# kevalmorabia97/CoVA-Web-Object-Detection

Hardware: AMD Instinct MI355X
Metric: webpages/sec fwd+bwd (90 bboxes, K=24) (higher is better)
Workload: dtype f32

## Files before the change

### cova-web-object-detection_amd/csrc/bn.hip

```cpp
#include "common.h"
#include "bn_tail.h"

namespace {

__device__ __forceinline__ int pow2_cols(int C)
{
    int cb = 1;
    while (cb < C && cb < 256) cb <<= 1;
    return cb;
}
inline int pow2_cols_host(int C)
{
    int cb = 1;
    while (cb < C && cb < 256) cb <<= 1;
    return cb;
}

template <int MODE>
__global__ __launch_bounds__(256) void colreduce_kernel(
    const float *__restrict__ x, int ldx, const float *__restrict__ act, int lda,
    const float *__restrict__ z, int ldz, const float *__restrict__ mean,
    const float *__restrict__ invstd, float *__restrict__ partial, long long R, int C,
    int rows_per_chunk)
{
// ... 180 lines not shown
        if (dbeta) dbeta[c] = (float)s1;
        if (dgamma) dgamma[c] = (float)s2;
        coef[c] = (float)(s1 / count);
        coef[C + c] = (float)(s2 / count);
    }
}

__global__ __launch_bounds__(1024) void bn_finalize_bwd_abc_kernel(
    const float *__restrict__ partial, int nparts, int C, double count,
    float *__restrict__ dgamma, float *__restrict__ dbeta, const float *__restrict__ mean,
    const float *__restrict__ invstd, const float *__restrict__ scale, float *__restrict__ abc)
{
    __shared__ double s_a[1024], s_b[1024];
    const int c = blockIdx.x * 64 + (threadIdx.x & 63), slice = threadIdx.x >> 6;
    double s1, s2;
    combine_partials(partial, nparts, C, c, slice, s_a, s_b, s1, s2);
    if (slice == 0 && c < C) bn_bwd_abc_channel(s1, s2, count, c, C, dgamma, dbeta, mean, invstd, scale, abc);
}

template <int V>
__global__ __launch_bounds__(256) void bn_act_fwd_kernel(
    const float *__restrict__ z, int ldz, const float *__restrict__ scale,
    const float *__restrict__ shift, const float *__restrict__ res, int ldres,
    float *__restrict__ out, int ldo, long long R, int C, int relu)
{
    const int CV = C / V;
    const long long total = R * CV;
    for (long long i = (long long)blockIdx.x * blockDim.x + threadIdx.x; i < total;
         i += (long long)gridDim.x * blockDim.x) {
        const long long r = i / CV;
        const int c = (int)(i - r * CV) * V;
        float v[V], sc[V], sh[V], rr[V];
        if (V == 4) {
            *reinterpret_cast<float4 *>(v) = *reinterpret_cast<const float4 *>(z + r * ldz + c);
            *reinterpret_cast<float4 *>(sc) = *reinterpret_cast<const float4 *>(scale + c);
            *reinterpret_cast<float4 *>(sh) = *reinterpret_cast<const float4 *>(shift + c);
            if (res) *reinterpret_cast<float4 *>(rr) = *reinterpret_cast<const float4 *>(res + r * ldres + c);
        } else {
            v[0] = z[r * ldz + c]; sc[0] = scale[c]; sh[0] = shift[c];
            if (res) rr[0] = res[r * ldres + c];
        }
#pragma unroll
        for (int j = 0; j < V; ++j) {
            float y = fmaf(sc[j], v[j], sh[j]);
            if (res) y += rr[j];
            if (relu) y = y > 0.f ? y : 0.f;
            v[j] = y;
        }
        if (V == 4) *reinterpret_cast<float4 *>(out + r * ldo + c) = *reinterpret_cast<float4 *>(v);
        else out[r * ldo + c] = v[0];
    }
}

template <int U>
__global__ __launch_bounds__(256) void bn_act_fwd_bits_kernel(
    const float *__restrict__ z, const float *__restrict__ scale, const float *__restrict__ shift,
    const float *__restrict__ res, float *__restrict__ out, uint32_t *__restrict__ bits, long long R)
{
    const long long total = R * 16;
    const long long stride = (long long)gridDim.x * blockDim.x;
    const int c = (int)(threadIdx.x & 15) * 4;
    const float4 sc = *reinterpret_cast<const float4 *>(scale + c), sh = *reinterpret_cast<const float4 *>(shift + c);
    for (long long i0 = (long long)blockIdx.x * blockDim.x + threadIdx.x; i0 < total; i0 += stride * U) {
      float4 vv[U], rr[U];
#pragma unroll
      for (int u = 0; u < U; ++u) {
        const long long i = i0 + u * stride;
        const long long ic = i < total ? i : i0;
        vv[u] = *reinterpret_cast<const float4 *>(z + ic * 4);
        if (res != nullptr) rr[u] = *reinterpret_cast<const float4 *>(res + ic * 4);
      }
#pragma unroll
      for (int u = 0; u < U; ++u) {
        const long long i = i0 + u * stride;
        if (i >= total) break;
        const float4 v = vv[u];
        float y[4] = {fmaf(sc.x, v.x, sh.x), fmaf(sc.y, v.y, sh.y), fmaf(sc.z, v.z, sh.z), fmaf(sc.w, v.w, sh.w)};
        if (res != nullptr) {
            const float4 r4 = rr[u];
            y[0] += r4.x; y[1] += r4.y; y[2] += r4.z; y[3] += r4.w;
        }
        uint32_t word = 0u;
#pragma unroll
        for (int j = 0; j < 4; ++j) {
            y[j] = y[j] > 0.f ? y[j] : 0.f;
            word |= (y[j] > 0.f ? 1u : 0u) << j;
        }
        *reinterpret_cast<float4 *>(out + i * 4) = make_float4(y[0], y[1], y[2], y[3]);
        word <<= 4 * (threadIdx.x & 7);
        word |= __shfl_xor(word, 1, 64);
        word |= __shfl_xor(word, 2, 64);
        word |= __shfl_xor(word, 4, 64);
        if ((threadIdx.x & 7) == 0) bits[i >> 3] = word;
      }
    }
}

__global__ __launch_bounds__(256) void bn_act2_fwd_kernel(
    const float *__restrict__ z, const float *__restrict__ scale, const float *__restrict__ shift,
    const float *__restrict__ z2, const float *__restrict__ scale2, const float *__restrict__ shift2,
    float *__restrict__ out, long long R, int C, int relu)
{
    const int CV = C / 4;
    const long long total = R * CV;
    for (long long i = (long long)blockIdx.x * blockDim.x + threadIdx.x; i < total;
         i += (long long)gridDim.x * blockDim.x) {
        const int c = (int)(i % CV) * 4;
        const float4 a = *reinterpret_cast<const float4 *>(z + i * 4);
        const float4 b = *reinterpret_cast<const float4 *>(z2 + i * 4);
        const float4 sa = *reinterpret_cast<const float4 *>(scale + c), ha = *reinterpret_cast<const float4 *>(shift + c);
        const float4 sb = *reinterpret_cast<const float4 *>(scale2 + c), hb = *reinterpret_cast<const float4 *>(shift2 + c);
        float4 y;
        y.x = fmaf(sa.x, a.x, ha.x) + fmaf(sb.x, b.x, hb.x);
        y.y = fmaf(sa.y, a.y, ha.y) + fmaf(sb.y, b.y, hb.y);
        y.z = fmaf(sa.z, a.z, ha.z) + fmaf(sb.z, b.z, hb.z);
        y.w = fmaf(sa.w, a.w, ha.w) + fmaf(sb.w, b.w, hb.w);
        if (relu) {
            y.x = y.x > 0.f ? y.x : 0.f; y.y = y.y > 0.f ? y.y : 0.f;
            y.z = y.z > 0.f ? y.z : 0.f; y.w = y.w > 0.f ? y.w : 0.f;
        }
        *reinterpret_cast<float4 *>(out + i * 4) = y;
    }
}

template <int V>
__global__ __launch_bounds__(256) void bn_bwd_apply_kernel(
    const float *__restrict__ dout, int ldd, const float *__restrict__ act, int lda,
    const float *__restrict__ z, int ldz, const float *__restrict__ mean,
    const float *__restrict__ invstd, const float *__restrict__ scale,
    const float *__restrict__ coef, float *__restrict__ dz, int lddz, float *__restrict__ dres,
    int lddres, long long R, int C)
{
    const int CV = C / V;
    const long long total = R * CV;
    for (long long i = (long long)blockIdx.x * blockDim.x + threadIdx.x; i < total;
         i += (long long)gridDim.x * blockDim.x) {
        const long long r = i / CV;
        const int c = (int)(i - r * CV) * V;
        float g[V], a[V], zz[V], o[V];
        if (V == 4) {
            *reinterpret_cast<float4 *>(g) = *reinterpret_cast<const float4 *>(dout + r * ldd + c);
            *reinterpret_cast<float4 *>(zz) = *reinterpret_cast<const float4 *>(z + r * ldz + c);
            if (act) *reinterpret_cast<float4 *>(a) = *reinterpret_cast<const float4 *>(act + r * lda + c);
        } else {
            g[0] = dout[r * ldd + c]; zz[0] = z[r * ldz + c];
            if (act) a[0] = act[r * lda + c];
        }
#pragma unroll
        for (int j = 0; j < V; ++j) {
            float dy = g[j];
            if (act && !(a[j] > 0.f)) dy = 0.f;
            g[j] = dy;
            const float xh = (zz[j] - mean[c + j]) * invstd[c + j];
            o[j] = scale[c + j] * (dy - coef[c + j] - xh * coef[C + c + j]);
        }
        if (V == 4) {
            *reinterpret_cast<float4 *>(dz + r * lddz + c) = *reinterpret_cast<float4 *>(o);
            if (dres) *reinterpret_cast<float4 *>(dres + r * lddres + c) = *reinterpret_cast<float4 *>(g);
        } else {
            dz[r * lddz + c] = o[0];
            if (dres) dres[r * lddres + c] = g[0];
        }
    }
}

template <bool XCD>
__global__ __launch_bounds__(256) void bn_relu_maxpool_fwd_kernel(
    const float *__restrict__ y, const float *__restrict__ scale, const float *__restrict__ shift,
    float *__restrict__ out, uint8_t *__restrict__ idx, float *__restrict__ ymax, int B, int H1, int W1,
    int H2, int W2)
{
    constexpr int POOL_STRIP = 1;
    const int nstrips = (H2 + POOL_STRIP - 1) / POOL_STRIP;
    const long long total = (long long)B * nstrips * W2 * 16;
    long long wb = blockIdx.x;
    if (XCD) {
        const long long per = gridDim.x / 8;
        if (wb < per * 8) wb = (wb % 8) * per + wb / 8;
    }
    for (long long i = wb * blockDim.x + threadIdx.x; i < total; i += (long long)gridDim.x * blockDim.x) {
        const int c4 = (int)(i & 15);
        long long p = i >> 4;
        const int ox = (int)(p % W2);
        p /= W2;
        const int strip = (int)(p % nstrips), b = (int)(p / nstrips);
        const float4 sc = *reinterpret_cast<const float4 *>(scale + c4 * 4);
        const float4 sh = *reinterpret_cast<const float4 *>(shift + c4 * 4);
        const float scv[4] = {sc.x, sc.y, sc.z, sc.w}, shv[4] = {sh.x, sh.y, sh.z, sh.w};
        const float *yb = y + (size_t)b * H1 * W1 * 64 + c4 * 4;
        const int ix0 = 2 * ox - 1;
        const bool okx[3] = {ix0 >= 0, true, ix0 + 2 < W1};
        auto load_row = [&](int iy, float4 (&r)[3]) {
#pragma unroll
            for (int kx = 0; kx < 3; ++kx) {
                const int ix = min(max(ix0 + kx, 0), W1 - 1), iyc = min(max(iy, 0), H1 - 1);
                r[kx] = *reinterpret_cast<const float4 *>(yb + ((size_t)iyc * W1 + ix) * 64);
            }
        };
        const int oy0 = strip * POOL_STRIP, oy1 = min(oy0 + POOL_STRIP, H2);
        float4 top[3], mid[3], bot[3];
        load_row(2 * oy0 - 1, top);
        for (int oy = oy0; oy < oy1; ++oy) {
            load_row(2 * oy, mid);
            load_row(2 * oy + 1, bot);
            const bool oky[3] = {2 * oy - 1 >= 0, true, 2 * oy + 1 < H1};
            float m[4] = {-INFINITY, -INFINITY, -INFINITY, -INFINITY};
            float my[4] = {0.f, 0.f, 0.f, 0.f};
            int mi[4] = {0, 0, 0, 0};
#pragma unroll
            for (int ky = 0; ky < 3; ++ky) {
                const float4 *row = ky == 0 ? top : ky == 1 ? mid : bot;
#pragma unroll
                for (int kx = 0; kx < 3; ++kx) {
                    if (!(oky[ky] && okx[kx])) continue;
                    const float vv[4] = {row[kx].x, row[kx].y, row[kx].z, row[kx].w};
#pragma unroll
                    for (int j = 0; j < 4; ++j) {
                        const float t = fmaf(vv[j], scv[j], shv[j]);
                        const float a = t > 0.f ? t : 0.f;
                        if (a > m[j]) { m[j] = a; mi[j] = ky * 3 + kx; my[j] = vv[j]; }
                    }
                }
            }
            const size_t o = (((size_t)b * H2 + oy) * W2 + ox) * 64 + c4 * 4;
            *reinterpret_cast<float4 *>(out + o) = make_float4(m[0], m[1], m[2], m[3]);
            *reinterpret_cast<uchar4 *>(idx + o) = make_uchar4(mi[0], mi[1], mi[2], mi[3]);
            if (ymax != nullptr) *reinterpret_cast<float4 *>(ymax + o) = make_float4(my[0], my[1], my[2], my[3]);
#pragma unroll
            for (int kx = 0; kx < 3; ++kx) top[kx] = bot[kx];
        }
    }
}

__global__ __launch_bounds__(256) void bn_relu_maxpool_bwd_reduce_win_kernel(
    const float *__restrict__ dp, const uint8_t *__restrict__ idx, const float *__restrict__ y,
    const float *__restrict__ scale, const float *__restrict__ shift,
    const float *__restrict__ mean, const float *__restrict__ invstd, float *__restrict__ partial,
    int B, int H1, int W1, int H2, int W2)
{
    __shared__ float s_s[16][64], s_q[16][64];
    const int c4 = threadIdx.x & 15, prow = threadIdx.x >> 4;
    const float4 sc = *reinterpret_cast<const float4 *>(scale + c4 * 4);
    const float4 sh = *reinterpret_cast<const float4 *>(shift + c4 * 4);
    const float4 mu = *reinterpret_cast<const float4 *>(mean + c4 * 4);
    const float4 is = *reinterpret_cast<const float4 *>(invstd + c4 * 4);
    const float scv[4] = {sc.x, sc.y, sc.z, sc.w}, shv[4] = {sh.x, sh.y, sh.z, sh.w};
    const float muv[4] = {mu.x, mu.y, mu.z, mu.w}, isv[4] = {is.x, is.y, is.z, is.w};
    float s[4] = {0, 0, 0, 0}, q[4] = {0, 0, 0, 0};
    const long long nwin = (long long)B * H2 * W2;
    for (long long p = (long long)blockIdx.x * 16 + prow; p < nwin; p += (long long)gridDim.x * 16) {
        const int ox = (int)(p % W2);
        const long long pr = p / W2;
        const int oy = (int)(pr % H2);
        const int b = (int)(pr / H2);
        const uchar4 id = *reinterpret_cast<const uchar4 *>(idx + (size_t)p * 64 + c4 * 4);
        const float4 g = *reinterpret_cast<const float4 *>(dp + (size_t)p * 64 + c4 * 4);
        const int pos[4] = {id.x, id.y, id.z, id.w};
        const float gv[4] = {g.x, g.y, g.z, g.w};
        const float *yb = y + (size_t)b * H1 * W1 * 64 + c4 * 4;
#pragma unroll
        for (int j = 0; j < 4; ++j) {
            const int ky = pos[j] / 3, kx = pos[j] - ky * 3;
            const int iy = 2 * oy - 1 + ky, ix = 2 * ox - 1 + kx;
            const float yv = yb[((size_t)iy * W1 + ix) * 64 + j];
            const float t = fmaf(yv, scv[j], shv[j]);
            const float dy = t > 0.f ? gv[j] : 0.f;
            s[j] += dy;
            q[j] += dy * ((yv - muv[j]) * isv[j]);
        }
    }
#pragma unroll
    for (int j = 0; j < 4; ++j) { s_s[prow][c4 * 4 + j] = s[j]; s_q[prow][c4 * 4 + j] = q[j]; }
    __syncthreads();
    if (threadIdx.x < 64) {
        float a = 0.f, bq = 0.f;
        for (int r = 0; r < 16; ++r) { a += s_s[r][threadIdx.x]; bq += s_q[r][threadIdx.x]; }
        partial[((size_t)blockIdx.x * 2 + 0) * 64 + threadIdx.x] = a;
        partial[((size_t)blockIdx.x * 2 + 1) * 64 + threadIdx.x] = bq;
// ... 119 lines not shown
                       (const float *)nullptr, 0, (const float *)nullptr, 0, (const float *)nullptr,
                       (const float *)nullptr, partial, R, C, rpc);
    COVA_LAUNCH_CHECK();
    return COVA_OK;
}

COVA_API int cova_bn_finalize_fwd(const float *partial, int nparts, int C, double count,
                                  const float *gamma, const float *beta, float *running_mean,
                                  float *running_var, long long *num_batches_tracked, float momentum,
                                  float eps, float *scale, float *shift, float *mean, float *invstd,
                                  void *stream)
{
    COVA_REQUIRE(partial && gamma && beta && scale && shift && mean && invstd && nparts > 0 && C > 0);
    hipLaunchKernelGGL(bn_finalize_fwd_kernel, dim3(cdiv(C, 64)), dim3(1024), 0, (hipStream_t)stream,
                       partial, nparts, C, count, gamma, beta, running_mean, running_var, momentum,
                       eps, scale, shift, mean, invstd, num_batches_tracked);
    COVA_LAUNCH_CHECK();
    return COVA_OK;
}

COVA_API int cova_bn_eval_params(const float *gamma, const float *beta, const float *running_mean,
                                 const float *running_var, float eps, int C, float *scale,
                                 float *shift, float *mean, float *invstd, void *stream)
{
    COVA_REQUIRE(gamma && beta && running_mean && running_var && scale && shift && C > 0);
    hipLaunchKernelGGL(bn_eval_params_kernel, dim3(cdiv(C, 256)), dim3(256), 0, (hipStream_t)stream,
                       gamma, beta, running_mean, running_var, eps, C, scale, shift, mean, invstd);
    COVA_LAUNCH_CHECK();
    return COVA_OK;
}

COVA_API int cova_bn_act_fwd(const float *z, int ldz, const float *scale, const float *shift,
                             const float *res, int ldres, float *out, int ldo, long long R, int C,
                             int relu, void *stream)
{
    COVA_REQUIRE(z && scale && shift && out && R > 0 && C > 0);
    const bool v4 = (C % 4 == 0) && vec4_ok(z, ldz) && vec4_ok(res, ldres) && vec4_ok(out, ldo) &&
                    vec4_ok(scale, 0) && vec4_ok(shift, 0);
    if (v4)
        hipLaunchKernelGGL(bn_act_fwd_kernel<4>, dim3(ew_grid(R * (C / 4))), dim3(256), 0,
                           (hipStream_t)stream, z, ldz, scale, shift, res, ldres, out, ldo, R, C, relu);
    else
        hipLaunchKernelGGL(bn_act_fwd_kernel<1>, dim3(ew_grid(R * C)), dim3(256), 0,
                           (hipStream_t)stream, z, ldz, scale, shift, res, ldres, out, ldo, R, C, relu);
    COVA_LAUNCH_CHECK();
    return COVA_OK;
}

COVA_API int cova_bn_act_fwd_bits(const float *z, const float *scale, const float *shift, const float *res, float *out,
                                  uint32_t *bits, long long R, void *stream)
{
    COVA_REQUIRE(z && scale && shift && out && bits && R > 0);
    COVA_REQUIRE(vec4_ok(z, 64) && vec4_ok(res, 64) && vec4_ok(out, 64) && vec4_ok(scale, 0) && vec4_ok(shift, 0));
    hipLaunchKernelGGL(bn_act_fwd_bits_kernel<1>, dim3(ew_grid(R * 16)), dim3(256), 0, (hipStream_t)stream, z, scale, shift,
                       res, out, bits, R);
    COVA_LAUNCH_CHECK();
    return COVA_OK;
}

COVA_API int cova_bn_act2_fwd(const float *z, const float *scale, const float *shift, const float *z2,
                              const float *scale2, const float *shift2, float *out, long long R, int C,
                              int relu, void *stream)
{
    COVA_REQUIRE(z && scale && shift && z2 && scale2 && shift2 && out && R > 0 && C > 0 && C % 4 == 0);
    COVA_REQUIRE(vec4_ok(z, C) && vec4_ok(z2, C) && vec4_ok(out, C) && vec4_ok(scale, 0) && vec4_ok(shift, 0) &&
                 vec4_ok(scale2, 0) && vec4_ok(shift2, 0));
    hipLaunchKernelGGL(bn_act2_fwd_kernel, dim3(ew_grid(R * (C / 4))), dim3(256), 0, (hipStream_t)stream, z,
                       scale, shift, z2, scale2, shift2, out, R, C, relu);
    COVA_LAUNCH_CHECK();
    return COVA_OK;
}

COVA_API int cova_bn_bwd_reduce(const float *dout, int ldd, const float *act, int lda,
                                const float *z, int ldz, const float *mean, const float *invstd,
                                long long R, int C, float *partial, void *stream)
{
    COVA_REQUIRE(dout && z && mean && invstd && partial && R > 0 && C > 0);
    const int rpc = cova_colreduce_rows_per_chunk(R, C);
    const dim3 grid((unsigned)cdivll(R, rpc), (unsigned)cdiv(C, pow2_cols_host(C)));
    if (C == 64 && ldd == 64 && ldz == 64 && (act == nullptr || lda == 64) && vec4_ok(dout, ldd) &&
        vec4_ok(z, ldz) && vec4_ok(act, lda)) {
        hipLaunchKernelGGL(colreduce64_kernel<1>, dim3(grid.x), dim3(256), 0, (hipStream_t)stream, dout,
                           act, z, mean, invstd, partial, R, rpc);
        COVA_LAUNCH_CHECK();
        return COVA_OK;
    }
    hipLaunchKernelGGL(colreduce_kernel<1>, grid, dim3(256), 0, (hipStream_t)stream, dout, ldd, act,
                       lda, z, ldz, mean, invstd, partial, R, C, rpc);
    COVA_LAUNCH_CHECK();
    return COVA_OK;
}

COVA_API int cova_bn_finalize_bwd(const float *partial, int nparts, int C, double count,
                                  float *dgamma, float *dbeta, float *coef, void *stream)
{
    COVA_REQUIRE(partial && coef && nparts > 0 && C > 0);
    hipLaunchKernelGGL(bn_finalize_bwd_kernel, dim3(cdiv(C, 64)), dim3(1024), 0, (hipStream_t)stream,
                       partial, nparts, C, count, dgamma, dbeta, coef);
    COVA_LAUNCH_CHECK();
    return COVA_OK;
}

COVA_API int cova_bn_finalize_bwd_abc(const float *partial, int nparts, int C, double count,
                                      float *dgamma, float *dbeta, const float *mean,
                                      const float *invstd, const float *scale, float *abc,
                                      void *stream)
{
    COVA_REQUIRE(partial && mean && invstd && scale && abc && nparts > 0 && C > 0);
    hipLaunchKernelGGL(bn_finalize_bwd_abc_kernel, dim3(cdiv(C, 64)), dim3(1024), 0,
                       (hipStream_t)stream, partial, nparts, C, count, dgamma, dbeta, mean, invstd,
                       scale, abc);
    COVA_LAUNCH_CHECK();
    return COVA_OK;
}

COVA_API int cova_bn_bwd_apply(const float *dout, int ldd, const float *act, int lda, const float *z,
                               int ldz, const float *mean, const float *invstd, const float *scale,
                               const float *coef, float *dz, int lddz, float *dres, int lddres,
                               long long R, int C, void *stream)
{
    COVA_REQUIRE(dout && z && mean && invstd && scale && coef && dz && R > 0 && C > 0);
    const bool v4 = (C % 4 == 0) && vec4_ok(dout, ldd) && vec4_ok(act, lda) && vec4_ok(z, ldz) &&
                    vec4_ok(dz, lddz) && vec4_ok(dres, lddres);
    if (v4)
        hipLaunchKernelGGL(bn_bwd_apply_kernel<4>, dim3(ew_grid(R * (C / 4))), dim3(256), 0,
                           (hipStream_t)stream, dout, ldd, act, lda, z, ldz, mean, invstd, scale,
                           coef, dz, lddz, dres, lddres, R, C);
    else
        hipLaunchKernelGGL(bn_bwd_apply_kernel<1>, dim3(ew_grid(R * C)), dim3(256), 0,
                           (hipStream_t)stream, dout, ldd, act, lda, z, ldz, mean, invstd, scale,
                           coef, dz, lddz, dres, lddres, R, C);
    COVA_LAUNCH_CHECK();
    return COVA_OK;
}

COVA_API int cova_bn_relu_maxpool_fwd(const float *y, const float *scale, const float *shift,
                                      float *out, uint8_t *idx, float *ymax, int B, int H1, int W1,
                                      void *stream)
{
    COVA_REQUIRE(y && scale && shift && out && idx && B > 0 && H1 > 0 && W1 > 0);
    const int H2 = (H1 + 2 - 3) / 2 + 1, W2 = (W1 + 2 - 3) / 2 + 1;
    long long g = cdivll((long long)B * H2 * W2 * 16, 256);
    if (g > 0x7fffffffll) g = 0x7fffffffll;
    hipLaunchKernelGGL(bn_relu_maxpool_fwd_kernel<true>, dim3((unsigned)g), dim3(256), 0, (hipStream_t)stream, y, scale, shift,
                       out, idx, ymax, B, H1, W1, H2, W2);
    COVA_LAUNCH_CHECK();
    return COVA_OK;
}

COVA_API int cova_bn_relu_maxpool_bwd_num_partials(int B, int H1, int W1)
{
    long long g = cdivll((long long)B * H1 * W1, 16 * 64);
    if (g > 4096) g = 4096;
    if (g < 1) g = 1;
    return (int)g;
}

COVA_API int cova_bn_relu_maxpool_bwd_reduce(const float *dp, const uint8_t *idx, const float *y,
                                             const float *scale, const float *shift,
                                             const float *mean, const float *invstd, float *partial,
                                             int B, int H1, int W1, void *stream)
{
    COVA_REQUIRE(dp && idx && y && scale && shift && mean && invstd && partial);
    const int H2 = (H1 + 2 - 3) / 2 + 1, W2 = (W1 + 2 - 3) / 2 + 1;
    const int grid = cova_bn_relu_maxpool_bwd_num_partials(B, H1, W1);
    hipLaunchKernelGGL(bn_relu_maxpool_bwd_reduce_win_kernel, dim3(grid), dim3(256), 0,
                       (hipStream_t)stream, dp, idx, y, scale, shift, mean, invstd, partial, B, H1, W1,
                       H2, W2);
    COVA_LAUNCH_CHECK();
    return COVA_OK;
}

COVA_API int cova_bn_relu_maxpool_bwd_apply(const float *dp, const uint8_t *idx, const float *y,
                                            const float *scale, const float *shift,
                                            const float *mean, const float *invstd,
                                            const float *coef, float *dz, int B, int H1, int W1,
                                            void *stream)
{
    COVA_REQUIRE(dp && idx && y && scale && shift && mean && invstd && coef && dz);
    const int H2 = (H1 + 2 - 3) / 2 + 1, W2 = (W1 + 2 - 3) / 2 + 1;
    const int grid = ew_grid((long long)B * H2 * W2 * 16);
    hipLaunchKernelGGL(bn_relu_maxpool_bwd_apply_quad_kernel, dim3(grid), dim3(256), 0,
                       (hipStream_t)stream, dp, idx, y, scale, shift, mean, invstd, coef, dz, B, H1, W1,
                       H2, W2);
    COVA_LAUNCH_CHECK();
    return COVA_OK;
}
```

### cova-web-object-detection_amd/engine.py

```python
import ctypes
import os

import torch

from . import _lib
from .weights import BACKBONE_CHANNELS as C64, CONTEXT_LAYERS, head_layout

GAT_MAX_K = 1024

call, query = _lib.call, _lib.query
BN_MOMENTUM, BN_EPS, LEAKY_SLOPE = 0.1, 1e-5, 0.2


DROPOUT_KEYS = ("decoder.0", "decoder.3")
ATTN_DROP_KEY = "attn_drop"
PAGE_ATTN_DROP_KEY = "page_attention.attn_drop"
PAGE_ENC_DROP_KEY = "page_encoder.drop"


def is_train(training, key):
    if isinstance(training, bool):
        return training
    if hasattr(training, "get"):
        return bool(training.get(key, True))
# ... 287 lines not shown
        self.c = c

    @property
    def ptr(self):
        return ctypes.addressof(self.c)


class Options:
    overlap_allreduce = os.environ.get("COVA_OVERLAP_ALLREDUCE", "1") != "0"
    bn_tail = os.environ.get("COVA_BN_TAIL", "1") != "0"


OPTIONS = Options()

CONV3_KEYS = ["convnet.4.0.conv1", "convnet.4.0.conv2", "convnet.4.1.conv1", "convnet.4.1.conv2"]
BN3_KEYS = ["convnet.4.0.bn1.", "convnet.4.0.bn2.", "convnet.4.1.bn1.", "convnet.4.1.bn2."]


class LazyFeature:
    __slots__ = ("z", "x", "scale", "shift", "shape")

    def __init__(self, z, x, scale, shift):
        self.z, self.x, self.scale, self.shift, self.shape = z, x, scale, shift, tuple(z.shape)


def is_bottleneck(params):
    return "convnet.4.0.conv3.weight" in params


@on_device_of(0)
def convstack_fwd(images, params, buffers, training, save=True, lazy_out=False):
    _check(images)
    B, _, H, W = images.shape
    H1, W1 = query("cova_conv_out_size", H, 7, 2, 3), query("cova_conv_out_size", W, 7, 2, 3)
    H2, W2 = query("cova_conv_out_size", H1, 3, 2, 1), query("cova_conv_out_size", W1, 3, 2, 1)
    bottleneck = is_bottleneck(params)
    layer2 = has_layer2(params)
    lazy_out = lazy_out and not layer2
    sv = {"images": images, "dims": (B, H, W, H1, W1, H2, W2), "kind": "bottleneck" if bottleneck else "basic"}
    if bottleneck:
        sv["_w3"] = conv3_weights([params["convnet.4.%d.conv2.weight" % b] for b in (0, 1, 2)], images)
    else:
        sv["_w3"] = conv3_weights([params[k + ".weight"] for k in CONV3_KEYS], images)
    y1 = _empty((B, H1, W1, C64), images)
    nt1 = query("cova_conv1_num_partials", B, H, W)
    stem_train = is_train(training, "convnet.1.")
    part = _empty((nt1, 2, C64), images) if stem_train else None
    if stem_train and tails_on():
        bn1, tail = bn_tail_fwd("convnet.1.", params, buffers, C64, images, B * H1 * W1)
        call("cova_conv1_fwd_tail", images, params["convnet.0.weight"], y1, part, B, H, W, tail.ptr)
    else:
        call("cova_conv1_fwd_tail", images, params["convnet.0.weight"], y1, part, B, H, W, None)
        bn1 = bn_params("convnet.1.", params, buffers, C64, images, training, part, nt1, B * H1 * W1, unit="pages")
    p1 = _empty((B, H2, W2, C64), images)
    idx = _empty((B, H2, W2, C64), images, torch.uint8)
    want_ymax = save and (stem_train or bottleneck)
    ymax = _empty((B, H2, W2, C64), images) if want_ymax else None
    call("cova_bn_relu_maxpool_fwd", y1, bn1.scale, bn1.shift, p1, idx, ymax, B, H1, W1)
    sv.update(y1=y1, bn1=bn1, idx=idx, ymax=ymax)
    if bottleneck:
        feat = _layer1_bottleneck_fwd(p1, params, buffers, training, save, lazy_out, sv)
    else:
        feat = _layer1_basic_fwd(p1, params, buffers, training, save, lazy_out, sv)
    if layer2:
        feat = _layer2_fwd(feat, params, buffers, training, save, sv)
    return feat, (sv if save else None)


def conv3_num_partials(B, H, W):
    return query("cova_conv3x3_wino4_num_partials", B, H, W)


def conv3x3_pro(u, inp, in2, abc, relu, addend, act, msc, msh, z, mean, invstd, out, part, B, H, W, tail=None,
                act_bits=None):
    if tail is not None:
        if act_bits is not None:
            act = None
        call("cova_conv3x3_wino4_full_tail", inp, in2, abc, relu, u, addend, act, act_bits, msc, msh, z, mean, invstd,
             out, part, B, H, W, tail.ptr)
    else:
        call("cova_conv3x3_wino4_full", inp, in2, abc, relu, u, addend, act, msc, msh, z, mean, invstd, out, part,
             B, H, W)


def conv3_weights(ws, like):
    n = len(ws)
    uf, ud = _empty((n, query("cova_conv3x3_wino4_u_floats")), like), _empty((n, query("cova_conv3x3_wino4_u_floats")), like)
    call("cova_conv3x3_wino4_prep_multi", *(list(ws) + [None] * (4 - n)), uf, ud)
    return [uf[i] for i in range(n)], [ud[i] for i in range(n)]


def conv_bn_fwd(u, inp, abc, relu, out, prefix, params, buffers, training, part, nt, R, B, H, W):
    training = is_train(training, prefix)
    if not training:
        part = None
    if training and tails_on():
        st, tail = bn_tail_fwd(prefix, params, buffers, C64, inp, R)
        conv3x3_pro(u, inp, None, abc, relu, None, None, None, None, None, None, None, out, part, B, H, W, tail)
        return st
    conv3x3_pro(u, inp, None, abc, relu, None, None, None, None, None, None, None, out, part, B, H, W)
    return bn_params(prefix, params, buffers, C64, inp, training, part, nt, R, unit="pages")


def conv_bn_pair_fwd(ua, ub, x, z1, z2, pa, pb, params, buffers, training, part, nt, R, B, H, W):
    bna = conv_bn_fwd(ua, x, None, 0, z1, pa, params, buffers, training, part, nt, R, B, H, W)
    bnb = conv_bn_fwd(ub, z1, bna.abc, 1, z2, pb, params, buffers, training, part, nt, R, B, H, W)
    return bna, bnb


def _layer1_basic_fwd(p1, params, buffers, training, save, lazy_out, sv):
    images = p1
    B, H, W, H1, W1, H2, W2 = sv["dims"]
    wf, wd = sv.pop("_w3")
    sv["wd"] = wd
    R = B * H2 * W2
    nt = conv3_num_partials(B, H2, W2)
    x = p1
    blocks = []
    for blk in (0, 1):
        ta, tb = is_train(training, BN3_KEYS[2 * blk]), is_train(training, BN3_KEYS[2 * blk + 1])
        if not save and not ta and not tb:
            bna = bn_params(BN3_KEYS[2 * blk], params, buffers, C64, images, False)
            bnb = bn_params(BN3_KEYS[2 * blk + 1], params, buffers, C64, images, False)
            ua, ub = wf[2 * blk], wf[2 * blk + 1]
            z1 = _empty((B, H2, W2, C64), images)
            call("cova_conv3x3_wino4", x, ua, z1, None, B, H2, W2)
            if blk == 1 and lazy_out:
                z2 = _empty((B, H2, W2, C64), images)
                call("cova_conv3x3_wino4_pro", z1, bna.abc, 1, ub, z2, None, B, H2, W2)
                feat = LazyFeature(z2, x, bnb.scale, bnb.shift)
                blocks.append(dict(x=x, z1=z1, a1=None, z2=z2, out=None, bna=bna, bnb=bnb))
                continue
            out = _empty((B, H2, W2, C64), images)
            call("cova_conv3x3_wino4_bnact", z1, bna.abc, 1, ub, x, bnb.scale, bnb.shift, 1, out, B, H2, W2)
            blocks.append(dict(x=x, z1=z1, a1=None, z2=None, out=out, bna=bna, bnb=bnb))
            x = feat = out
            continue
        part = _empty((nt, 2, C64), images) if ta or tb else None
        z1, z2 = _empty((B, H2, W2, C64), images), _empty((B, H2, W2, C64), images)
        bna, bnb = conv_bn_pair_fwd(wf[2 * blk], wf[2 * blk + 1], x, z1, z2, BN3_KEYS[2 * blk], BN3_KEYS[2 * blk + 1],
                                    params, buffers, training, part, nt, R, B, H2, W2)
        out_bits = None
        if blk == 1 and lazy_out:
            out = None
            feat = LazyFeature(z2, x, bnb.scale, bnb.shift)
        else:
            out = _empty((B, H2, W2, C64), images)
            if blk == 0 and save and tb and tails_on():
                out_bits = _empty((R, 2), images, torch.int32)
                call("cova_bn_act_fwd_bits", z2, bnb.scale, bnb.shift, x, out, out_bits, R)
            else:
                call("cova_bn_act_fwd", z2, C64, bnb.scale, bnb.shift, x, C64, out, C64, R, C64, 1)
            feat = out
        blocks.append(dict(x=x, z1=z1, a1=None, z2=z2, out=out, bna=bna, bnb=bnb, out_bits=out_bits))
        x = out
    sv["blocks"] = blocks
    last = blocks[1]
    sv["last"] = dict(out=last["out"], x=last["x"], z=last["z2"], bn=last["bnb"], prefix=BN3_KEYS[3])
    return feat


C256 = 4 * C64


def conv1x1(inp, in2, abc, relu, w, w_trans, out, part, R, cin, cout, addend=None, act=None, msc=None,
            msh=None, z=None, mean=None, invstd=None, z2=None, mean2=None, invstd2=None, part2=None, act_bits=None):
    call("cova_conv1x1", inp, in2, abc, 1 if relu else 0, w, 1 if w_trans else 0, addend, act, act_bits, msc, msh,
         z, mean, invstd, z2, mean2, invstd2, out, part, part2, R, cin, cout)


def _layer1_bottleneck_fwd(p1, params, buffers, training, save, lazy_out, sv):
    B, H, W, H1, W1, H2, W2 = sv["dims"]
    R = B * H2 * W2
    nt = conv3_num_partials(B, H2, W2)

    def stats(cin, cout, prefix):
        n = query("cova_conv1x1_num_partials", R, cin, cout)
        return (_empty((n, 2, cout), p1) if is_train(training, prefix) else None), n

    def bn(prefix, C, part, n):
        return bn_params(prefix, params, buffers, C, p1, training, part, n, R, unit="pages")

    ufs, uds = sv.pop("_w3")
    x, cin, blocks, feat = p1, C64, [], None
    pending = None
    for blk in (0, 1, 2):
        pre = "convnet.4.%d." % blk
        s = dict(cin=cin, pre=pre)
        part, n = stats(cin, C64, pre + "bn1.")
        s["z1"] = _empty((B, H2, W2, C64), p1)
        if pending is None:
            conv1x1(x, None, None, 0, params[pre + "conv1.weight"], 0, s["z1"], part, R, cin, C64)
        else:
            x = _empty((B, H2, W2, C256), p1)
            s["x_bits"] = (_empty((R, C256 // 32), p1, torch.int32)
                           if save and is_train(training, "convnet.4.%d.bn3." % (blk - 1)) else None)
            call("cova_conv1x1_materialize", pending[0], pending[1], pending[2], params[pre + "conv1.weight"], x,
                 s["x_bits"], s["z1"], part, R)
            blocks[-1]["out"] = x
        s["x"] = x
        s["bn1"] = bn(pre + "bn1.", C64, part, n)
        uf, s["ud"] = ufs[blk], uds[blk]
        part = _empty((nt, 2, C64), p1) if is_train(training, pre + "bn2.") else None
        s["z2"] = _empty((B, H2, W2, C64), p1)
        s["bn2"] = conv_bn_fwd(uf, s["z1"], s["bn1"].abc, 1, s["z2"], pre + "bn2.", params, buffers, training, part, nt,
                               R, B, H2, W2)
        part, n = stats(C64, C256, pre + "bn3.")
        s["z3"] = _empty((B, H2, W2, C256), p1)
# ... 180 lines not shown
def _layer1_bwd_fused(sv, dfeat, gout, grads, head_part=None, plan=None):
    if plan is None:
        plan = frozenset(["stem"] + ["wgrad:%s.weight" % k for k in CONV3_KEYS])
    B, H, W, H1, W1, H2, W2 = sv["dims"]
    R = B * H2 * W2
    wg = "cova_conv3x3_wgrad4"
    nws = query("cova_conv3x3_wgrad4_workspace_floats", B, H2, W2)
    wanted = [k for k in CONV3_KEYS if "wgrad:%s.weight" % k in plan]
    ws_all = _empty((len(wanted), nws), dfeat) if wanted else None
    jobs = {}

    def wgrad(key, act, act_abc, act_relu, dz, dz2, dz_abc, side=True):
        if key not in wanted:
            return None
        dw = _gbuf(gout, key + ".weight", (64, 64, 3, 3), dfeat)
        out = torch.empty_like(dz) if dz_abc is not None and side else None
        ws = ws_all[len(jobs)]
        call(wg + "_partial", act, act_abc, act_relu, dz, dz2, dz_abc, out, ws, B, H2, W2)
        jobs[3 - CONV3_KEYS.index(key)] = (ws, dw)
        grads[key + ".weight"] = dw
        return out

    nt = conv3_num_partials(B, H2, W2)
    dA, pend = dfeat, None
    if isinstance(head_part, dict):
        pend = head_part["pend"]
    elif head_part is not None:
        last = sv["blocks"][1]["bnb"]
        pend = _bn_abc_from_partials(head_part[0], head_part[1], last, R, gout, BN3_KEYS[3], dfeat)
    for blk in (1, 0):
        s = sv["blocks"][blk]
        ka, kb = CONV3_KEYS[2 * blk], CONV3_KEYS[2 * blk + 1]
        pa, pb = BN3_KEYS[2 * blk], BN3_KEYS[2 * blk + 1]
        bna, bnb = s["bna"], s["bnb"]
        if pend is None:
            dres, dz2 = torch.empty_like(dA), torch.empty_like(dA)
            dg, db = bn_backward(dA, C64, block_out(s), C64, s["z2"], C64, bnb, R, dz2, C64, dres, C64,
                                 gout, pb, unit="pages")
            g_in, g_in2, g_abc = dz2, None, None
        else:
            dres = dA
            dg, db, g_abc = pend
            g_in, g_in2 = dA, s["z2"]
        grads[pb + "weight"], grads[pb + "bias"] = dg, db
        dzm = wgrad(kb, s["z1"], bna.abc, 1, g_in, g_in2, g_abc)
        if dzm is not None:
            g_in, g_in2, g_abc = dzm, None, None
        dy_a = torch.empty_like(dA)
        part = _empty((nt, 2, C64), dfeat)
        dg, db, abc_a = dgrad_bn_bwd(sv["wd"][2 * blk + 1], g_in, g_in2, g_abc, None, None, bna.scale, bna.shift, s["z1"],
                                     bna, dy_a, part, nt, R, gout, pa, B, H2, W2)
        grads[pa + "weight"], grads[pa + "bias"] = dg, db
        last_dgrad = blk == 1 or "stem" in plan
        dzm = wgrad(ka, s["x"], None, 0, dy_a, s["z1"], abc_a, side=last_dgrad)
        if not last_dgrad:
            dA = None
            break
        d_in, d_in2, d_abc = (dy_a, s["z1"], abc_a) if dzm is None else (dzm, None, None)
        dx = torch.empty_like(dA)
        if blk == 1:
            prev = sv["blocks"][0]
            pend = dgrad_bn_bwd(sv["wd"][2 * blk], d_in, d_in2, d_abc, dres, prev["out"], None, None, prev["z2"],
                                prev["bnb"], dx, _empty((nt, 2, C64), dfeat), nt, R, gout, BN3_KEYS[1], B, H2, W2,
                                act_bits=prev.get("out_bits"))
        elif sv.get("ymax") is not None:
            bn1 = sv["bn1"]
            sv["pool_abc"] = dgrad_bn_bwd(sv["wd"][2 * blk], d_in, d_in2, d_abc, dres, None, bn1.scale, bn1.shift,
                                          sv["ymax"], bn1, dx, _empty((nt, 2, C64), dfeat), nt, B * H1 * W1, gout,
                                          "convnet.1.", B, H2, W2)
        else:
            conv3x3_pro(sv["wd"][2 * blk], d_in, d_in2, d_abc, 0, dres, None, None, None, None, None, None, dx,
                        None, B, H2, W2)
        dA = dx
    if jobs:
        fin = []
        for i in range(4):
            fin += list(jobs.get(i, (None, None)))
        call(wg + "_finish", *fin, B, H2, W2)
    return dA


C128 = 2 * C64
L2 = "convnet.5."
L2_CONVS = [(L2 + "0.conv1", C64, 3, 2, 1), (L2 + "0.conv2", C128, 3, 1, 1), (L2 + "0.downsample.0", C64, 1, 2, 0),
            (L2 + "1.conv1", C128, 3, 1, 1), (L2 + "1.conv2", C128, 3, 1, 1)]


def conv_nhwc_prep(w, fwd=True, dgrad=True):
    co, ci, k, _ = w.shape
    wf = _empty((k * k * ci, co), w) if fwd else None
    wd = _empty((k * k * co, ci), w) if dgrad else None
    call("cova_conv_nhwc_prep", w, wf, wd, co, ci, k)
    return wf, wd


def _layer2_fwd(x, params, buffers, training, save, sv):
    B, H2, W2, _ = x.shape
    H3, W3 = query("cova_conv_out_size", H2, 3, 2, 1), query("cova_conv_out_size", W2, 3, 2, 1)
    R = B * H3 * W3
    ops = {key: conv_nhwc_prep(params[key + ".weight"], dgrad=save) for key, *_ in L2_CONVS}
    geo = {key: rest for key, *rest in L2_CONVS}

    def conv(inp, key):
        ci, k, s, p = geo[key]
        out = _empty((B, H3, W3, C128), x)
        call("cova_conv_nhwc_fwd", inp, ops[key][0], out, B, inp.shape[1], inp.shape[2], ci, C128, k, s, p)
        return out
# ... 1185 lines not shown
```

### include/cova_hip.h

```cpp
#ifndef COVA_HIP_H
#define COVA_HIP_H

#include <stdint.h>

#ifdef __cplusplus
extern "C" {
#endif

#define COVA_ERR_BAD_ARG 10001

typedef struct cova_bn_tail {
    int mode;
    int *counter;
    double count;
    const float *gamma, *beta;
    float *running_mean, *running_var;
    long long *num_batches_tracked;
    float momentum, eps;
    float *scale, *shift, *mean, *invstd;
    float *dgamma, *dbeta, *abc;
} cova_bn_tail;

int cova_conv_out_size(int in_size, int kernel, int stride, int pad);
int cova_set_option(int key, int value);
// ... 67 lines not shown
int cova_conv1x1_materialize(const float *in, const float *in2, const float *pro_abc , const float *w,
                             float *side, uint32_t *side_bits, float *out, float *stat_part , long long R,
                             void *stream);
int cova_conv1x1_wgrad_workspace_floats(long long R, int Co, int Ci);
int cova_conv1x1_wgrad(const float *dz, const float *dz2 , const float *dz_abc ,
                       const float *act, const float *act_abc , int act_relu, float *dw,
                       float *ws, long long R, int Co, int Ci, void *stream);

int cova_conv1x1_lin_floats(void);
int cova_conv1x1_vprod_workspace_floats(long long R);
int cova_conv1x1_vprod(const float *v, const float *act, const float *act_abc , int act_relu,
                       float *lin, float *ws, long long R, void *stream);
int cova_conv1x1_lin_bnsums(const float *lin, const float *w, const float *mean, const float *invstd,
                            float *part, void *stream);
int cova_conv1x1_lin_finish(const float *lin, const float *abc, const float *w, float *dw, float *m,
                            float *cvec, float *avec, void *stream);
int cova_conv1x1_lin_dgrad_num_partials(long long R);
int cova_conv1x1_lin_dgrad(const float *v, const float *avec, const float *w, const float *act,
                           const float *act_abc, int act_relu, const float *m, const float *cvec,
                           const float *addend , const float *mask_scale,
                           const float *mask_shift, const float *z, const float *mean, const float *invstd,
                           float *out, float *stat_part, long long R, void *stream);

int cova_conv_nhwc_prep(const float *w_oihw, float *w_fwd, float *w_dgrad, int Co, int Ci, int k, void *stream);
int cova_conv_nhwc_fwd(const float *in, const float *w_fwd, float *out, int B, int H, int W, int Ci, int Co, int k,
                       int stride, int pad, void *stream);
int cova_conv_nhwc_dgrad(const float *dy, const float *w_dgrad, const float *dy2, const float *w2_dgrad,
                         const float *addend, float *dx, int B, int H, int W, int Ci, int Co, int k, int stride, int pad,
                         void *stream);
int cova_conv_nhwc_wgrad_num_partials(int B, int Ho, int Wo, int Ci, int Co, int k);
int cova_conv_nhwc_wgrad_workspace_floats(int B, int Ho, int Wo, int Ci, int Co, int k);
int cova_conv_nhwc_wgrad(const float *in, const float *dy, float *dw, float *ws, int B, int H, int W, int Ci, int Co,
                         int k, int stride, int pad, void *stream);

int cova_partials_fold(const float *partial, int nparts, int width, int group, float *out,
                       void *stream);
int cova_colreduce_rows_per_chunk(long long R, int C);
int cova_colreduce_num_chunks(long long R, int C);
int cova_colstats(const float *x, int ldx, long long R, int C, float *partial ,
                  void *stream);
int cova_bn_finalize_fwd(const float *partial, int nparts, int C, double count, const float *gamma,
                         const float *beta, float *running_mean , float *running_var,
                         long long *num_batches_tracked ,
                         float momentum, float eps, float *scale, float *shift, float *mean,
                         float *invstd, void *stream);
int cova_bn_eval_params(const float *gamma, const float *beta, const float *running_mean,
                        const float *running_var, float eps, int C, float *scale, float *shift,
                        float *mean , float *invstd , void *stream);
int cova_bn_act_fwd(const float *z, int ldz, const float *scale, const float *shift,
                    const float *res , int ldres, float *out, int ldo, long long R, int C,
                    int relu, void *stream);
int cova_bn_act_fwd_bits(const float *z, const float *scale, const float *shift, const float *res, float *out,
                         uint32_t *bits, long long R, void *stream);
int cova_bn_act2_fwd(const float *z, const float *scale, const float *shift, const float *z2,
                     const float *scale2, const float *shift2, float *out, long long R, int C, int relu,
                     void *stream);
int cova_bn_bwd_reduce(const float *dout, int ldd, const float *act ,
                       int lda, const float *z, int ldz, const float *mean, const float *invstd,
                       long long R, int C, float *partial , void *stream);
int cova_bn_finalize_bwd(const float *partial, int nparts, int C, double count,
                         float *dgamma , float *dbeta , float *coef ,
                         void *stream);
int cova_bn_finalize_bwd_abc(const float *partial, int nparts, int C, double count,
                             float *dgamma , float *dbeta , const float *mean,
                             const float *invstd, const float *scale, float *abc, void *stream);
int cova_bn_bwd_apply(const float *dout, int ldd, const float *act, int lda, const float *z, int ldz,
                      const float *mean, const float *invstd, const float *scale, const float *coef,
                      float *dz, int lddz, float *dres , int lddres, long long R, int C,
                      void *stream);
int cova_bn1d_fwd(const float *x, int ldx, int R, int C, const float *gamma, const float *beta,
                  float *running_mean , float *running_var, long long *num_batches_tracked ,
                  float momentum, float eps, int relu, float *out, int ldo, float *dropped , int ld_dropped,
                  uint8_t *mask, float p, unsigned long long seed, int mask_given, float *scale, float *shift,
                  float *mean, float *invstd, void *stream);
int cova_bn1d_bwd(const float *dout, int ldg, const uint8_t *drop_mask , float p,
                  const float *act , int lda, const float *z, int ldz, const float *mean,
                  const float *invstd, const float *scale, int R, int C, float *dgamma, float *dbeta, float *dz,
                  int lddz, float *dz_colsum , void *stream);
int cova_bn_relu_maxpool_fwd(const float *y , const float *scale, const float *shift,
                             float *out , uint8_t *idx,
                             float *ymax , int B, int H1,
                             int W1, void *stream);
int cova_bn_relu_maxpool_bwd_num_partials(int B, int H1, int W1);
int cova_bn_relu_maxpool_bwd_reduce(const float *dp, const uint8_t *idx, const float *y,
                                    const float *scale, const float *shift, const float *mean,
                                    const float *invstd, float *partial, int B, int H1, int W1,
                                    void *stream);
int cova_bn_relu_maxpool_bwd_apply(const float *dp, const uint8_t *idx, const float *y,
                                   const float *scale, const float *shift, const float *mean,
                                   const float *invstd, const float *coef, float *dz, int B, int H1,
                                   int W1, void *stream);

int cova_roipool_fwd(const float *feat, const float *rois, int n_rois, int B, int C, int H, int W,
                     int PH, int PW, float spatial_scale, float *out, int ld_out, int32_t *argmax,
                     void *stream);
int cova_roipool_bwd(const float *gout, int ld_g, const float *rois, const int32_t *argmax,
                     int n_rois, int B, int C, int H, int W, int PH, int PW, float spatial_scale,
                     float *gfeat, void *ws , void *stream);
int cova_roipool_bwd_workspace_words(int n_rois, int B, int C, int PH, int PW);
int cova_roipool_bwd_bn_num_partials(int n_rois);
int cova_roipool_bwd_bn(const float *gout, int ld_g, const float *pooled, int ld_p, const float *zmax,
                        const float *rois, const int32_t *argmax, int n_rois, int B, int C, int H, int W,
                        int PH, int PW, float spatial_scale, const float *mean, const float *invstd,
                        float *gfeat, float *partial, void *ws ,
                        void *stream);
int cova_roipool_bwd_bn_tail(const float *gout, int ld_g, const float *pooled, int ld_p, const float *zmax,
// ... 220 lines not shown
```

Measured before the change: 1812.

## Skip materializing pooled stem output; recompute BN+ReLU of ymax in consumers

When training with the basic layer1 and tails enabled, the stem maxpool no longer writes the pooled activation map p1. Downstream consumers (first conv, residual add in bits kernel, weight-grad) instead read the raw pre-BN max values (ymax) and apply the stem BN affine plus ReLU on the fly. This removes one full feature-map write and its later reads, at the cost of extra FMAs in consumers and more template variants.

```diff
diff --git a/cova-web-object-detection_amd/csrc/bn.hip b/cova-web-object-detection_amd/csrc/bn.hip
--- a/cova-web-object-detection_amd/csrc/bn.hip
+++ b/cova-web-object-detection_amd/csrc/bn.hip
@@ -256,15 +256,18 @@
     }
 }
 
-template <int U>
+template <int U, bool RAW>
 __global__ __launch_bounds__(256) void bn_act_fwd_bits_kernel(
     const float *__restrict__ z, const float *__restrict__ scale, const float *__restrict__ shift,
-    const float *__restrict__ res, float *__restrict__ out, uint32_t *__restrict__ bits, long long R)
+    const float *__restrict__ res, const float *__restrict__ res_scale, const float *__restrict__ res_shift, int res_relu,
+    float *__restrict__ out, uint32_t *__restrict__ bits, long long R)
 {
     const long long total = R * 16;
     const long long stride = (long long)gridDim.x * blockDim.x;
     const int c = (int)(threadIdx.x & 15) * 4;
     const float4 sc = *reinterpret_cast<const float4 *>(scale + c), sh = *reinterpret_cast<const float4 *>(shift + c);
+    float4 rsc = make_float4(0.f, 0.f, 0.f, 0.f), rsh = rsc;
+    if (RAW) { rsc = *reinterpret_cast<const float4 *>(res_scale + c); rsh = *reinterpret_cast<const float4 *>(res_shift + c); }
     for (long long i0 = (long long)blockIdx.x * blockDim.x + threadIdx.x; i0 < total; i0 += stride * U) {
       float4 vv[U], rr[U];
 #pragma unroll
@@ -281,7 +284,14 @@
         const float4 v = vv[u];
         float y[4] = {fmaf(sc.x, v.x, sh.x), fmaf(sc.y, v.y, sh.y), fmaf(sc.z, v.z, sh.z), fmaf(sc.w, v.w, sh.w)};
         if (res != nullptr) {
-            const float4 r4 = rr[u];
+            float4 r4 = rr[u];
+            if (RAW) {
+                r4 = make_float4(fmaf(rsc.x, r4.x, rsh.x), fmaf(rsc.y, r4.y, rsh.y), fmaf(rsc.z, r4.z, rsh.z), fmaf(rsc.w, r4.w, rsh.w));
+                if (res_relu) {
+                    r4.x = r4.x > 0.f ? r4.x : 0.f; r4.y = r4.y > 0.f ? r4.y : 0.f;
+                    r4.z = r4.z > 0.f ? r4.z : 0.f; r4.w = r4.w > 0.f ? r4.w : 0.f;
+                }
+            }
             y[0] += r4.x; y[1] += r4.y; y[2] += r4.z; y[3] += r4.w;
         }
         uint32_t word = 0u;
@@ -368,7 +378,7 @@
     }
 }
 
-template <bool XCD>
+template <bool XCD, bool OUT>
 __global__ __launch_bounds__(256) void bn_relu_maxpool_fwd_kernel(
     const float *__restrict__ y, const float *__restrict__ scale, const float *__restrict__ shift,
     float *__restrict__ out, uint8_t *__restrict__ idx, float *__restrict__ ymax, int B, int H1, int W1,
@@ -427,7 +437,7 @@
                 }
             }
             const size_t o = (((size_t)b * H2 + oy) * W2 + ox) * 64 + c4 * 4;
-            *reinterpret_cast<float4 *>(out + o) = make_float4(m[0], m[1], m[2], m[3]);
+            if (OUT) *reinterpret_cast<float4 *>(out + o) = make_float4(m[0], m[1], m[2], m[3]);
             *reinterpret_cast<uchar4 *>(idx + o) = make_uchar4(mi[0], mi[1], mi[2], mi[3]);
             if (ymax != nullptr) *reinterpret_cast<float4 *>(ymax + o) = make_float4(my[0], my[1], my[2], my[3]);
 #pragma unroll
@@ -653,8 +663,21 @@
 {
     COVA_REQUIRE(z && scale && shift && out && bits && R > 0);
     COVA_REQUIRE(vec4_ok(z, 64) && vec4_ok(res, 64) && vec4_ok(out, 64) && vec4_ok(scale, 0) && vec4_ok(shift, 0));
-    hipLaunchKernelGGL(bn_act_fwd_bits_kernel<1>, dim3(ew_grid(R * 16)), dim3(256), 0, (hipStream_t)stream, z, scale, shift,
-                       res, out, bits, R);
+    hipLaunchKernelGGL((bn_act_fwd_bits_kernel<1, false>), dim3(ew_grid(R * 16)), dim3(256), 0, (hipStream_t)stream, z, scale, shift,
+                       res, nullptr, nullptr, 0, out, bits, R);
+    COVA_LAUNCH_CHECK();
+    return COVA_OK;
+}
+
+COVA_API int cova_bn_act_fwd_bits_res(const float *z, const float *scale, const float *shift, const float *res_raw,
+                                      const float *res_scale, const float *res_shift, int res_relu, float *out,
+                                      uint32_t *bits, long long R, void *stream)
+{
+    COVA_REQUIRE(z && scale && shift && res_raw && res_scale && res_shift && out && bits && R > 0);
+    COVA_REQUIRE(vec4_ok(z, 64) && vec4_ok(res_raw, 64) && vec4_ok(out, 64) && vec4_ok(scale, 0) && vec4_ok(shift, 0) &&
+                 vec4_ok(res_scale, 0) && vec4_ok(res_shift, 0));
+    hipLaunchKernelGGL((bn_act_fwd_bits_kernel<1, true>), dim3(ew_grid(R * 16)), dim3(256), 0, (hipStream_t)stream, z, scale, shift,
+                       res_raw, res_scale, res_shift, res_relu, out, bits, R);
     COVA_LAUNCH_CHECK();
     return COVA_OK;
 }
@@ -739,12 +762,16 @@
                                       float *out, uint8_t *idx, float *ymax, int B, int H1, int W1,
                                       void *stream)
 {
-    COVA_REQUIRE(y && scale && shift && out && idx && B > 0 && H1 > 0 && W1 > 0);
+    COVA_REQUIRE(y && scale && shift && (out || ymax) && idx && B > 0 && H1 > 0 && W1 > 0);
     const int H2 = (H1 + 2 - 3) / 2 + 1, W2 = (W1 + 2 - 3) / 2 + 1;
     long long g = cdivll((long long)B * H2 * W2 * 16, 256);
     if (g > 0x7fffffffll) g = 0x7fffffffll;
-    hipLaunchKernelGGL(bn_relu_maxpool_fwd_kernel<true>, dim3((unsigned)g), dim3(256), 0, (hipStream_t)stream, y, scale, shift,
-                       out, idx, ymax, B, H1, W1, H2, W2);
+    if (out)
+        hipLaunchKernelGGL((bn_relu_maxpool_fwd_kernel<true, true>), dim3((unsigned)g), dim3(256), 0, (hipStream_t)stream, y, scale,
+                           shift, out, idx, ymax, B, H1, W1, H2, W2);
+    else
+        hipLaunchKernelGGL((bn_relu_maxpool_fwd_kernel<true, false>), dim3((unsigned)g), dim3(256), 0, (hipStream_t)stream, y, scale,
+                           shift, out, idx, ymax, B, H1, W1, H2, W2);
     COVA_LAUNCH_CHECK();
     return COVA_OK;
 }
diff --git a/cova-web-object-detection_amd/engine.py b/cova-web-object-detection_amd/engine.py
--- a/cova-web-object-detection_amd/engine.py
+++ b/cova-web-object-detection_amd/engine.py
@@ -363,12 +363,14 @@
     else:
         call("cova_conv1_fwd_tail", images, params["convnet.0.weight"], y1, part, B, H, W, None)
         bn1 = bn_params("convnet.1.", params, buffers, C64, images, training, part, nt1, B * H1 * W1, unit="pages")
-    p1 = _empty((B, H2, W2, C64), images)
     idx = _empty((B, H2, W2, C64), images, torch.uint8)
     want_ymax = save and (stem_train or bottleneck)
     ymax = _empty((B, H2, W2, C64), images) if want_ymax else None
+    single_map = (want_ymax and not bottleneck and not layer2 and tails_on()
+                  and is_train(training, BN3_KEYS[1]))
+    p1 = None if single_map else _empty((B, H2, W2, C64), images)
     call("cova_bn_relu_maxpool_fwd", y1, bn1.scale, bn1.shift, p1, idx, ymax, B, H1, W1)
-    sv.update(y1=y1, bn1=bn1, idx=idx, ymax=ymax)
+    sv.update(y1=y1, bn1=bn1, idx=idx, ymax=ymax, p1=p1)
     if bottleneck:
         feat = _layer1_bottleneck_fwd(p1, params, buffers, training, save, lazy_out, sv)
     else:
@@ -413,20 +415,20 @@
     return bn_params(prefix, params, buffers, C64, inp, training, part, nt, R, unit="pages")
 
 
-def conv_bn_pair_fwd(ua, ub, x, z1, z2, pa, pb, params, buffers, training, part, nt, R, B, H, W):
-    bna = conv_bn_fwd(ua, x, None, 0, z1, pa, params, buffers, training, part, nt, R, B, H, W)
+def conv_bn_pair_fwd(ua, ub, x, z1, z2, pa, pb, params, buffers, training, part, nt, R, B, H, W, x_abc=None, x_relu=0):
+    bna = conv_bn_fwd(ua, x, x_abc, x_relu, z1, pa, params, buffers, training, part, nt, R, B, H, W)
     bnb = conv_bn_fwd(ub, z1, bna.abc, 1, z2, pb, params, buffers, training, part, nt, R, B, H, W)
     return bna, bnb
 
 
 def _layer1_basic_fwd(p1, params, buffers, training, save, lazy_out, sv):
-    images = p1
+    x, x_abc, x_relu = (p1, None, 0) if p1 is not None else (sv["ymax"], sv["bn1"].abc, 1)
+    images = x
     B, H, W, H1, W1, H2, W2 = sv["dims"]
     wf, wd = sv.pop("_w3")
     sv["wd"] = wd
     R = B * H2 * W2
     nt = conv3_num_partials(B, H2, W2)
-    x = p1
     blocks = []
     for blk in (0, 1):
         ta, tb = is_train(training, BN3_KEYS[2 * blk]), is_train(training, BN3_KEYS[2 * blk + 1])
@@ -450,7 +452,7 @@
         part = _empty((nt, 2, C64), images) if ta or tb else None
         z1, z2 = _empty((B, H2, W2, C64), images), _empty((B, H2, W2, C64), images)
         bna, bnb = conv_bn_pair_fwd(wf[2 * blk], wf[2 * blk + 1], x, z1, z2, BN3_KEYS[2 * blk], BN3_KEYS[2 * blk + 1],
-                                    params, buffers, training, part, nt, R, B, H2, W2)
+                                    params, buffers, training, part, nt, R, B, H2, W2, x_abc, x_relu)
         out_bits = None
         if blk == 1 and lazy_out:
             out = None
@@ -459,12 +461,17 @@
             out = _empty((B, H2, W2, C64), images)
             if blk == 0 and save and tb and tails_on():
                 out_bits = _empty((R, 2), images, torch.int32)
-                call("cova_bn_act_fwd_bits", z2, bnb.scale, bnb.shift, x, out, out_bits, R)
+                if x_abc is not None:
+                    call("cova_bn_act_fwd_bits_res", z2, bnb.scale, bnb.shift, x, x_abc[0], x_abc[2], x_relu, out, out_bits, R)
+                else:
+                    call("cova_bn_act_fwd_bits", z2, bnb.scale, bnb.shift, x, out, out_bits, R)
             else:
+                assert x_abc is None
                 call("cova_bn_act_fwd", z2, C64, bnb.scale, bnb.shift, x, C64, out, C64, R, C64, 1)
             feat = out
-        blocks.append(dict(x=x, z1=z1, a1=None, z2=z2, out=out, bna=bna, bnb=bnb, out_bits=out_bits))
-        x = out
+        blocks.append(dict(x=x, x_abc=x_abc, x_relu=x_relu, z1=z1, a1=None, z2=z2, out=out, bna=bna, bnb=bnb,
+                           out_bits=out_bits))
+        x, x_abc, x_relu = out, None, 0
     sv["blocks"] = blocks
     last = blocks[1]
     sv["last"] = dict(out=last["out"], x=last["x"], z=last["z2"], bn=last["bnb"], prefix=BN3_KEYS[3])
@@ -751,7 +758,7 @@
                                      bna, dy_a, part, nt, R, gout, pa, B, H2, W2)
         grads[pa + "weight"], grads[pa + "bias"] = dg, db
         last_dgrad = blk == 1 or "stem" in plan
-        dzm = wgrad(ka, s["x"], None, 0, dy_a, s["z1"], abc_a, side=last_dgrad)
+        dzm = wgrad(ka, s["x"], s.get("x_abc"), s.get("x_relu", 0), dy_a, s["z1"], abc_a, side=last_dgrad)
         if not last_dgrad:
             dA = None
             break
diff --git a/include/cova_hip.h b/include/cova_hip.h
--- a/include/cova_hip.h
+++ b/include/cova_hip.h
@@ -143,6 +143,9 @@
                     int relu, void *stream);
 int cova_bn_act_fwd_bits(const float *z, const float *scale, const float *shift, const float *res, float *out,
                          uint32_t *bits, long long R, void *stream);
+int cova_bn_act_fwd_bits_res(const float *z, const float *scale, const float *shift, const float *res_raw,
+                             const float *res_scale, const float *res_shift, int res_relu, float *out,
+                             uint32_t *bits, long long R, void *stream);
 int cova_bn_act2_fwd(const float *z, const float *scale, const float *shift, const float *z2,
                      const float *scale2, const float *shift2, float *out, long long R, int C, int relu,
                      void *stream);
```

Result: no change. 1822 (median of 6 runs) (+0.6%).
